# VinAIResearch/Point-Unet

Measured on AMD Instinct MI355X. Metric: points_per_sec_forward, higher is better.
Workload: dtype f32

## Files before the change

point-unet_amd/csrc/debug_hooks.h:

```cpp
#ifndef POINTSEG_DEBUG_H
#define POINTSEG_DEBUG_H
#include "../../include/pointseg.h"
#ifdef __cplusplus
extern "C" {
#endif
int ps_debug_knn_host(const float* support, const float* queries, int64_t B, int64_t n_support,
                      int64_t n_queries, int64_t K, int32_t* out_idx);
int ps_debug_kdtree_host(const float* support, int64_t n, int32_t* vind, int32_t* nodes, float* pts,
                         int32_t* root_depth, float* bbox);
int ps_debug_kdtree_device(ps_context* ctx, const float* support, int64_t n, int32_t* vind, int32_t* nodes,
                           float* pts, int32_t* root_depth, float* bbox);
int ps_debug_pack_weights(const float* W, int cin, int cout, int ntb, float* out);
int ps_debug_pack_b3(const float* W, int cin, int cout, uint16_t* out);
int ps_debug_gemm32(ps_context* ctx, int split_bf16, const float* x1, int ld1, int c1, const int32_t* g1, const float* x2, int ld2, int c2,
                    const int32_t* g2, int gm, int gn, const float* W, const float* bias, int64_t R, int cout, int leaky, float* y, int ldy);
int ps_debug_gemm32_plan(ps_context* ctx, int split_bf16, int64_t R, int cin, int cout, int* out4);

int ps_debug_set_tuning(ps_context* ctx, const char* field, double value);
int ps_debug_get_tuning(ps_context* ctx, const char* field, double* value);
int ps_debug_tuning_fields(char* buf, int cap);
int ps_debug_volume_sample_args_size(void);

#ifdef __cplusplus
}
#endif
#endif
```

point-unet_amd/csrc/debug_hooks.hip:

```cpp
#include "common.h"

#include <cstring>
#include <vector>
#include "kdtree_build.h"
#include "kdtree_host.h"
#include "rowgemm.h"
#include "attpool.h"

using namespace ps;

extern "C" int ps_debug_volume_sample_args_size(void) { return (int)sizeof(ps_volume_sample_args); }

extern "C" int ps_debug_pack_weights(const float* W, int cin, int cout, int ntb, float* out)
{
    PS_CHECK(W && out && (ntb == 1 || ntb == 2 || ntb == 4), "ps_debug_pack_weights: bad argument");
    pack_weights(W, cin, cout, ntb, out);
    return PS_OK;
}

extern "C" int ps_debug_pack_b3(const float* W, int cin, int cout, uint16_t* out)
{
    PS_CHECK(W && out && cin > 0 && cin % 32 == 0 && cout > 0 && cout % 32 == 0, "ps_debug_pack_b3: bad argument");
    pack_b3(W, cin, cout, out);
    return PS_OK;
}

extern "C" int ps_debug_gemm32(ps_context* c, int split_bf16, const float* x1, int ld1, int c1, const int32_t* g1, const float* x2, int ld2, int c2,
                               const int32_t* g2, int gm, int gn, const float* W, const float* bias, int64_t R, int cout, int leaky, float* y, int ldy)
{
    PS_CHECK(c && x1 && W && bias && y && R >= 0 && c1 > 0 && c2 >= 0 && cout > 0, "ps_debug_gemm32: bad argument");
    PS_HIP(hipSetDevice(c->device));
    const int cin = c1 + c2;
    PS_CHECK(cin % (split_bf16 ? 16 : 8) == 0 && cout % 32 == 0, "ps_debug_gemm32: cin %% %d and cout %% 32 must be 0", split_bf16 ? 16 : 8);
    std::vector<float> img((size_t)cin * cout * (split_bf16 ? 3 : 2) / 2);
    if (split_bf16) pack_p32b(W, cin, cout, reinterpret_cast<uint16_t*>(img.data()));
    else pack_p32(W, cin, cout, img.data());
    float *d_img = nullptr, *d_bias = nullptr;
    PS_HIP(hipMalloc(reinterpret_cast<void**>(&d_img), img.size() * sizeof(float)));
    PS_HIP(hipMalloc(reinterpret_cast<void**>(&d_bias), sizeof(float) * (size_t)cout));
    PS_HIP(hipMemcpyAsync(d_img, img.data(), img.size() * sizeof(float), hipMemcpyHostToDevice, c->stream));
    PS_HIP(hipMemcpyAsync(d_bias, bias, sizeof(float) * (size_t)cout, hipMemcpyHostToDevice, c->stream));
    PackedLinear L;
    L.cin = cin; L.cout = cout; L.leaky = leaky; L.bias = d_bias;
    if (split_bf16) L.w32b = d_img; else L.w32 = d_img;
    RowSrc s1, s2;
    s1.x = x1; s1.ld = ld1; s1.c = c1; s1.gather = g1; s1.gm = g1 ? gm : 0; s1.gn = g1 ? gn : 0;
    s2.x = x2; s2.ld = ld2; s2.c = c2; s2.gather = g2; s2.gm = g2 ? gm : 0; s2.gn = g2 ? gn : 0;
    int rc = PS_EINVAL;
    if (split_bf16 ? gemm32b_fits(L, s1, s2, R, ldy) : gemm32_fits(L, s1, s2, R, ldy))
        rc = split_bf16 ? gemm32b(c, L, s1, s2, R, y, ldy) : gemm32(c, L, s1, s2, R, y, ldy);
    else
        set_error("ps_debug_gemm32: the shape does not fit the kernel");
    (void)hipStreamSynchronize(c->stream);
    (void)hipFree(d_img);
    (void)hipFree(d_bias);
    return rc;
}

extern "C" int ps_debug_gemm32_plan(ps_context* c, int split_bf16, int64_t R, int cin, int cout, int* out4)
{
    PS_CHECK(c && out4 && R >= 1 && cin > 0 && cout > 0 && cin % (split_bf16 ? 16 : 8) == 0 && cout % 32 == 0, "ps_debug_gemm32_plan: bad argument");
    const Gemm32Plan p = split_bf16 ? gemm32b_plan(c->tune, R, cin, cout) : gemm32_plan(c->tune, R, cin, cout);
    out4[0] = p.rw;
    out4[1] = p.cw;
    out4[2] = p.sk;
    out4[3] = p.pd;
    return PS_OK;
}

static bool is_bool(double v) { return v == 0 || v == 1; }
static bool is_int_in(double v, double lo, double hi) { return v >= lo && v <= hi && v == (double)(int64_t)v; }

#define PS_TUNING_FIELDS(X)                                                \
    X(gemm32b_min_flops, v >= 0 && v <= 1e300)                             \
    X(gemm32b_rw, v == 0 || v == 1 || v == 2)                              \
    X(gemm32b_cw, v == 0 || v == 1 || v == 2)                              \
    X(gemm32_no_sk8, is_bool(v))                                           \
    X(att64_gemm, is_bool(v))                                              \
    X(att64_occ, v == 0 || v == 1 || v == 2)                               \
    X(att_no_split, is_bool(v))                                            \
    X(wgrad_b3_min_rows, is_int_in(v, 0, (double)(1ll << 40)))             \
    X(gemm_b3_min_rows, is_int_in(v, 0, (double)(1ll << 40)))              \
    X(wgrad_wgs, is_int_in(v, 64, 4096))                                   \
    X(bn_slice, is_bool(v))                                                \
    X(inv_bucket, is_bool(v))                                              \
    X(inv_tile, v == 4096 || v == 6144 || v == 8192)                       \
    X(gather_reduce_ordered, is_bool(v))                                   \
    X(maxpool_bwd_ordered, is_bool(v))                                     \
    X(train_act_bf16, is_bool(v))                                          \
    X(train_att_gemm_split, v == -1 || v == 0 || v == 1)                   \
    X(train_att_gemm, is_bool(v))                                          \
    X(train_att128_fwd_gemm, is_bool(v))                                   \
    X(train_fuse_residual, is_bool(v))                                     \
    X(train_merge_syncbn, is_bool(v))                                      \
    X(convbn_max_c, is_int_in(v, 0, 4096))                                 \
    X(convbn_rect_max, is_int_in(v, 0, (double)(1 << 30)))                 \
    X(wgrad_debug, is_bool(v))

extern "C" int ps_debug_set_tuning(ps_context* c, const char* field, double v)
{
    PS_CHECK(c && field, "ps_debug_set_tuning: NULL argument");
#define PS_SET(f, ok)                                                                                 \
    if (std::strcmp(field, #f) == 0) {                                                                \
        PS_CHECK(ok, "ps_debug_set_tuning: %g is not a value %s is compiled for", v, #f);             \
        c->tune.f = static_cast<decltype(c->tune.f)>(v);                                              \
        return PS_OK;                                                                                 \
    }
    PS_TUNING_FIELDS(PS_SET)
#undef PS_SET
    PS_CHECK(false, "ps_debug_set_tuning: no knob named '%s'", field);
}

extern "C" int ps_debug_get_tuning(ps_context* c, const char* field, double* out)
{
    PS_CHECK(c && field && out, "ps_debug_get_tuning: NULL argument");
#define PS_GET(f, ok)                               \
    if (std::strcmp(field, #f) == 0) {              \
        *out = static_cast<double>(c->tune.f);      \
        return PS_OK;                               \
    }
    PS_TUNING_FIELDS(PS_GET)
#undef PS_GET
    PS_CHECK(false, "ps_debug_get_tuning: no knob named '%s'", field);
}

extern "C" int ps_debug_tuning_fields(char* buf, int cap)
{
    static const char names[] =
#define PS_NAME(f, ok) #f "\n"
        PS_TUNING_FIELDS(PS_NAME)
#undef PS_NAME
        ;
    PS_CHECK(buf && cap >= (int)sizeof(names), "ps_debug_tuning_fields: need %d bytes", (int)sizeof(names));
    std::memcpy(buf, names, sizeof(names));
    return PS_OK;
}

extern "C" int ps_debug_kdtree_device(ps_context* c, const float* support, int64_t n, int32_t* vind, int32_t* nodes, float* pts,
                                      int32_t* root_depth, float* bbox)
{
    PS_CHECK(c && support && vind && nodes && pts && root_depth && bbox && n >= 1, "ps_debug_kdtree_device: bad argument");
    PS_HIP(hipSetDevice(c->device));
    PS_TRY(c->stage_in.reserve(sizeof(float) * 3 * (size_t)n));
    PS_HIP(hipMemcpyAsync(c->stage_in.p, support, sizeof(float) * 3 * (size_t)n, hipMemcpyHostToDevice, c->stream));
    TreeSetPlan plan;
    plan.add((int32_t)n);
    for (int pass = 0; pass < 2; ++pass) {
        c->knn_arena.begin(pass == 0);
        plan.carve(c->knn_arena);
        if (pass == 0) PS_TRY(c->knn_arena.buf.reserve(c->knn_arena.off));
    }
    plan.src[0] = c->stage_in.as<float>();
    PS_TRY(build_trees(c, plan));
    int32_t flag[3] = {0, 0, 0};
    PS_HIP(hipMemcpyAsync(flag, plan.d_flags, 12, hipMemcpyDeviceToHost, c->stream));
    PS_HIP(hipStreamSynchronize(c->stream));
    PS_CHECK(flag[1] == 0, "ps_debug_kdtree_device: builder queue overflow");
    TreeMeta m;
    PS_HIP(hipMemcpyAsync(nodes, plan.d_nodes[0], sizeof(int4) * 2 * (size_t)n, hipMemcpyDeviceToHost, c->stream));
    PS_HIP(hipMemcpyAsync(pts, plan.d_pts[0], sizeof(float4) * (size_t)n, hipMemcpyDeviceToHost, c->stream));
    PS_HIP(hipMemcpyAsync(&m, plan.d_meta, sizeof(TreeMeta), hipMemcpyDeviceToHost, c->stream));
    PS_HIP(hipStreamSynchronize(c->stream));
    for (int64_t i = 0; i < n; ++i) std::memcpy(&vind[i], &pts[4 * i + 3], 4);
    root_depth[0] = m.root;
    root_depth[1] = m.depth;
    for (int a = 0; a < 3; ++a) {
        bbox[a] = m.lo[a];
        bbox[3 + a] = m.hi[a];
    }
    return PS_OK;
}
```

point-unet_amd/csrc/regchain.hip:

```cpp
#include <algorithm>

#include "mfma_tile.h"
#include "rowgemm.h"

namespace ps {

struct RcLayer {
    const float* wp;
    const float* bias;
    float* y;
    const float* ex;
    int ca, cb;
    int ta, tb;
    int cout, ot;
    int ks, ntb;
    int ldy, ldex, leaky;
    int w_off, b_off;
};
struct RcArgs {
    const float* x1; const int32_t* g1; int ld1, g1m, g1n;
    const float* x2; const int32_t* g2; int ld2, g2m, g2n;
    int n, R;
    RcLayer l[kChainMaxSteps];
    const float* image;
    int image_floats;
};

template <int N_, int A0_, int B0_, int O0_, int B1_ = 0, int O1_ = 0, int B2_ = 0, int O2_ = 0, int B3_ = 0, int O3_ = 0>
struct RcShape {
    static constexpr int N = N_, A0 = A0_;
    static constexpr int B[4] = {B0_, B1_, B2_, B3_};
    static constexpr int O[4] = {O0_, O1_, O2_, O3_};
    static constexpr int A(int l) { return l == 0 ? A0_ : O[l - 1]; }
    static constexpr int IN(int l) { return A(l) + B[l]; }
    static constexpr int maxt()
    {
        int m = 1;
        for (int l = 0; l < N_; ++l) {
            m = IN(l) > m ? IN(l) : m;
            m = O[l] > m ? O[l] : m;
        }
        return m;
    }
};

template <int T0, int NT, int MT>
__device__ __forceinline__ void rc_load(float (&dst)[MT][4], const float* __restrict__ rowp, int c, bool vec, int g)
{
#pragma unroll
    for (int t = 0; t < NT; ++t) {
        const int ch = t * 16 + 4 * g;
        if (vec) {
            float4 v = make_float4(0.f, 0.f, 0.f, 0.f);
            if (t + 1 < NT || ch < c) v = *reinterpret_cast<const float4*>(rowp + ch);
            dst[T0 + t][0] = v.x; dst[T0 + t][1] = v.y; dst[T0 + t][2] = v.z; dst[T0 + t][3] = v.w;
        } else {
#pragma unroll
            for (int q = 0; q < 4; ++q) dst[T0 + t][q] = (t + 1 < NT || ch + q < c) ? rowp[ch + q] : 0.f;
        }
    }
}

template <class S, int L>
__device__ __forceinline__ void rc_layer(const RcArgs& a, float (&act)[S::maxt()][4], const float* lds, int lane, int g, int row, int rr, bool ok)
{
    if constexpr (L < S::N) {
        constexpr int IT = S::IN(L), OT = S::O[L], TA = S::A(L), TB = S::B[L];
        const RcLayer& y = a.l[L];
        if constexpr (L > 0 && TB > 0) {
            const bool ve = (y.cb & 3) == 0 && (y.ldex & 3) == 0 && (reinterpret_cast<uintptr_t>(y.ex) & 15) == 0;
            rc_load<TA, TB>(act, y.ex + (size_t)rr * y.ldex, y.cb, ve, g);
        }
        f32x4 acc[OT];
#pragma unroll
        for (int to = 0; to < OT; ++to) acc[to] = f32x4{0.f, 0.f, 0.f, 0.f};
        if constexpr (L > 0) __builtin_amdgcn_sched_barrier(0);
        const float* w = lds + y.w_off + lane;
#pragma unroll
        for (int t0 = 0; t0 < OT; t0 += 4) {
#pragma unroll
            for (int ti = 0; ti < IT; ++ti)
#pragma unroll
                for (int q = 0; q < 4; ++q)
#pragma unroll
                    for (int to = t0; to < (t0 + 4 < OT ? t0 + 4 : OT); ++to)
                        acc[to] = __builtin_amdgcn_mfma_f32_16x16x4f32(w[((to * IT + ti) * 4 + q) * 64], act[ti][q], acc[to], 0, 0, 0);
            if (t0 + 4 < OT) __builtin_amdgcn_sched_barrier(0);
        }
        const bool vy = y.y && (y.cout & 3) == 0 && (y.ldy & 3) == 0 && (reinterpret_cast<uintptr_t>(y.y) & 15) == 0;
#pragma unroll
        for (int to = 0; to < OT; ++to) {
            const int ch = to * 16 + 4 * g;
            const float4 b = *reinterpret_cast<const float4*>(lds + y.b_off + ch);
            float v[4] = {acc[to][0] + b.x, acc[to][1] + b.y, acc[to][2] + b.z, acc[to][3] + b.w};
#pragma unroll
            for (int q = 0; q < 4; ++q) {
                if (y.leaky) v[q] = leaky02(v[q]);
                act[to][q] = v[q];
            }
            if (y.y && ok) {
                float* o = y.y + (size_t)row * y.ldy + ch;
                if (vy) {
                    if (to + 1 < OT || ch < y.cout) *reinterpret_cast<float4*>(o) = make_float4(v[0], v[1], v[2], v[3]);
                } else {
#pragma unroll
                    for (int q = 0; q < 4; ++q)
                        if (to + 1 < OT || ch + q < y.cout) o[q] = v[q];
                }
            }
        }
        rc_layer<S, L + 1>(a, act, lds, lane, g, row, rr, ok);
    }
}

__device__ __forceinline__ void rc_stage(const RcArgs& a, float* dst)
{
    for (int l = 0; l < a.n; ++l) {
        const RcLayer& y = a.l[l];
        const int it_n = y.ta + y.tb;
        const int ln = threadIdx.x & 63, q = threadIdx.x >> 6;
        const int i = ln & 15, gg = ln >> 4;
        const int npairs = it_n * y.ot;
        for (int base = 0; base < npairs; base += 8) {
            float v[8];
#pragma unroll
            for (int u = 0; u < 8; ++u) {
                const int pr = base + u;
                v[u] = 0.f;
                if (pr < npairs) {
                    const int ti = pr / y.ot, to = pr - ti * y.ot;
                    int k;
                    bool kok;
                    if (ti < y.ta) { k = ti * 16 + 4 * gg + q; kok = k < y.ca; }
                    else { k = (ti - y.ta) * 16 + 4 * gg + q; kok = k < y.cb; k += y.ca; }
                    const int cblk = to / y.ntb, j = to - cblk * y.ntb;
                    if (kok && to * 16 + i < y.cout) v[u] = y.wp[(((size_t)cblk * y.ks + (k >> 2)) * 64 + ((k & 3) * 16 + i)) * y.ntb + j];
                }
            }
#pragma unroll
            for (int u = 0; u < 8; ++u) {
                const int pr = base + u;
                if (pr < npairs) {
                    const int ti = pr / y.ot, to = pr - ti * y.ot;
                    dst[y.w_off + ((to * it_n + ti) * 4 + q) * 64 + ln] = v[u];
                }
            }
        }
        for (int e = threadIdx.x; e < y.ot * 16; e += 256) dst[y.b_off + e] = e < y.cout ? y.bias[e] : 0.f;
    }
}

__global__ __launch_bounds__(256) void rc_pack_kernel(RcArgs a, float* out) { rc_stage(a, out); }

template <class S>
__global__ __launch_bounds__(256) void regchain_kernel(RcArgs a)
{
    extern __shared__ __attribute__((aligned(16))) float rc_lds[];
    constexpr int MT = S::maxt();
    const int wave = threadIdx.x >> 6, lane = threadIdx.x & 63;
    const int p = lane & 15, g = lane >> 4;
    if (a.image) {
        for (int i = threadIdx.x; i < a.image_floats / 4; i += 256) reinterpret_cast<float4*>(rc_lds)[i] = reinterpret_cast<const float4*>(a.image)[i];
    } else {
        rc_stage(a, rc_lds);
    }
    __syncthreads();

    const bool v1 = (a.l[0].ca & 3) == 0 && (a.ld1 & 3) == 0 && (reinterpret_cast<uintptr_t>(a.x1) & 15) == 0;
    const bool v2 = (a.l[0].cb & 3) == 0 && (a.ld2 & 3) == 0 && (reinterpret_cast<uintptr_t>(a.x2) & 15) == 0;
    const int stride = gridDim.x * 4;
    auto load_inputs = [&](int tile, float (&dst)[MT][4]) {
        const int rr = min(tile * 16 + p, a.R - 1);
        const int s1 = a.g1 ? (a.g1m ? (rr / a.g1m) * a.g1n : 0) + a.g1[rr] : rr;
        rc_load<0, S::A0>(dst, a.x1 + (size_t)s1 * a.ld1, a.l[0].ca, v1, g);
        if constexpr (S::B[0] > 0) {
            const int s2 = a.g2 ? (a.g2m ? (rr / a.g2m) * a.g2n : 0) + a.g2[rr] : rr;
            rc_load<S::A0, S::B[0]>(dst, a.x2 + (size_t)s2 * a.ld2, a.l[0].cb, v2, g);
        }
    };
    int tile = blockIdx.x * 4 + wave;
    float act[MT][4], nxt[MT][4];
    if (tile * 16 < a.R) load_inputs(tile, nxt);
    for (; tile * 16 < a.R; tile += stride) {
#pragma unroll
        for (int t = 0; t < S::IN(0); ++t)
#pragma unroll
            for (int q = 0; q < 4; ++q) act[t][q] = nxt[t][q];
        if ((tile + stride) * 16 < a.R) load_inputs(tile + stride, nxt);
        const int row = tile * 16 + p;
        rc_layer<S, 0>(a, act, rc_lds, lane, g, row, min(row, a.R - 1), row < a.R);
    }
}

static inline int rc_tiles(int c) { return (c + 15) / 16; }

using RcFc0 = RcShape<2, 1, 0, 1, 0, 1>;
using RcEnc0 = RcShape<2, 1, 0, 1, 1, 2>;
using RcOne0 = RcShape<1, 1, 0, 1>;
using RcPair1 = RcShape<2, 2, 0, 2, 0, 4>;
using RcPair1b = RcShape<2, 4, 0, 2, 0, 4>;
using RcEnc1 = RcShape<2, 4, 0, 4, 2, 8>;
using RcPair2 = RcShape<2, 8, 0, 4, 0, 8>;
using RcHead = RcShape<4, 2, 2, 2, 0, 4, 0, 2, 0, 1>;

template <class S>
static bool rc_matches(const RcArgs& a)
{
    if (a.n != S::N) return false;
    for (int l = 0; l < S::N; ++l)
        if (a.l[l].ta != S::A(l) || a.l[l].tb != S::B[l] || a.l[l].ot != S::O[l]) return false;
    return true;
}

static bool rc_build(const ChainStep* steps, int n_steps, const RowSrc& s1, const RowSrc& s2, RcArgs& a, size_t& lds_bytes)
{
    if (n_steps < 1 || n_steps > kChainMaxSteps) return false;
    a = RcArgs{};
    a.x1 = s1.x; a.g1 = s1.gather; a.ld1 = s1.ld; a.g1m = s1.gm; a.g1n = s1.gn;
    a.x2 = s2.x; a.g2 = s2.gather; a.ld2 = s2.ld; a.g2m = s2.gm; a.g2n = s2.gn;
    a.n = n_steps;
    int off = 0, prev = 0;
    for (int i = 0; i < n_steps; ++i) {
        const PackedLinear* L = steps[i].L;
        if (!L || !L->wp || !L->bias) return false;
        if (steps[i].extra.x && (i == 0 || steps[i].extra.gather)) return false;
        RcLayer& y = a.l[i];
        y.wp = L->wp; y.bias = L->bias; y.y = steps[i].y; y.ldy = steps[i].ldy;
        y.ex = i > 0 ? steps[i].extra.x : nullptr; y.ldex = steps[i].extra.ld;
        y.ca = i == 0 ? s1.c : prev;
        y.cb = i == 0 ? s2.c : (steps[i].extra.x ? steps[i].extra.c : 0);
        if (y.ca + y.cb != L->cin) return false;
        y.ta = rc_tiles(y.ca); y.tb = rc_tiles(y.cb);
        y.cout = L->cout; y.ot = rc_tiles(L->cout);
        y.ks = L->ks; y.ntb = L->ntb; y.leaky = L->leaky;
        y.w_off = off; off += y.ot * (y.ta + y.tb) * 256;
        y.b_off = off; off += y.ot * 16;
        prev = L->cout;
    }
    lds_bytes = (size_t)off * sizeof(float);
    return rc_matches<RcFc0>(a) || rc_matches<RcEnc0>(a) || rc_matches<RcOne0>(a) || rc_matches<RcPair1>(a) || rc_matches<RcPair1b>(a) ||
           rc_matches<RcEnc1>(a) || rc_matches<RcPair2>(a) || rc_matches<RcHead>(a);
}

bool regchain_fits(const ChainStep* steps, int n_steps, const RowSrc& s1, const RowSrc& s2)
{
    RcArgs a;
    size_t lds = 0;
    return rc_build(steps, n_steps, s1, s2, a, lds);
}

template <class S>
static int rc_launch(ps_context* c, const RcArgs& a, size_t lds_bytes, int blocks)
{
    size_t& have = c->regchain_lds_attr[reinterpret_cast<const void*>(regchain_kernel<S>)];
    if (lds_bytes > 48 * 1024 && lds_bytes > have) {
        PS_HIP(hipFuncSetAttribute(reinterpret_cast<const void*>(regchain_kernel<S>), hipFuncAttributeMaxDynamicSharedMemorySize, (int)lds_bytes));
        have = lds_bytes;
    }
    hipLaunchKernelGGL(regchain_kernel<S>, dim3(blocks), dim3(256), lds_bytes, c->stream, a);
    return PS_OK;
}

int regchain(ps_context* c, const ChainStep* steps, int n_steps, const RowSrc& s1, const RowSrc& s2, int64_t R, ChainCache* cache)
{
    if (R <= 0) return PS_OK;
    RcArgs a;
    size_t lds_bytes = 0;
    PS_CHECK(rc_build(steps, n_steps, s1, s2, a, lds_bytes), "regchain: not one of the compiled chain shapes");
    PS_CHECK(R < (int64_t)1 << 31, "regchain: too many rows");
    a.R = (int)R;
    if (cache) {
        ChainCache::Entry* hit = nullptr;
        for (auto& e : cache->entries)
            if (e.wp0 == a.l[0].wp && e.wp_last == a.l[n_steps - 1].wp && e.n == n_steps && e.ca == a.l[0].ca && e.cb == a.l[0].cb) hit = &e;
        if (!hit) {
            cache->entries.emplace_back();
            hit = &cache->entries.back();
            hit->wp0 = a.l[0].wp; hit->wp_last = a.l[n_steps - 1].wp; hit->n = n_steps; hit->ca = a.l[0].ca; hit->cb = a.l[0].cb;
            PS_TRY(hit->img.reserve(lds_bytes));
            hipLaunchKernelGGL(rc_pack_kernel, dim3(1), dim3(256), 0, c->stream, a, hit->img.as<float>());
            PS_HIP(hipGetLastError());
        }
        a.image = hit->img.as<float>();
        a.image_floats = (int)(lds_bytes / sizeof(float));
    }
    const int tiles = (int)((R + 15) / 16);
    const int per_cu = std::max(1, std::min(4, (int)(160 * 1024 / std::max<size_t>(lds_bytes, 1))));
    const int blocks = std::max(1, std::min((tiles + 3) / 4, 256 * per_cu));
    if (rc_matches<RcFc0>(a)) PS_TRY(rc_launch<RcFc0>(c, a, lds_bytes, blocks));
    else if (rc_matches<RcEnc0>(a)) PS_TRY(rc_launch<RcEnc0>(c, a, lds_bytes, blocks));
    else if (rc_matches<RcOne0>(a)) PS_TRY(rc_launch<RcOne0>(c, a, lds_bytes, blocks));
    else if (rc_matches<RcPair1>(a)) PS_TRY(rc_launch<RcPair1>(c, a, lds_bytes, blocks));
    else if (rc_matches<RcPair1b>(a)) PS_TRY(rc_launch<RcPair1b>(c, a, lds_bytes, blocks));
    else if (rc_matches<RcEnc1>(a)) PS_TRY(rc_launch<RcEnc1>(c, a, lds_bytes, blocks));
    else if (rc_matches<RcPair2>(a)) PS_TRY(rc_launch<RcPair2>(c, a, lds_bytes, blocks));
    else PS_TRY(rc_launch<RcHead>(c, a, lds_bytes, blocks));
    PS_HIP(hipGetLastError());
    return PS_OK;
}

}
```

point-unet_amd/csrc/rowgemm.h:

```cpp
#pragma once

#include <vector>

#include "common.h"

namespace ps {

struct PackedLinear {
    const float* wp = nullptr;
    const float* wq = nullptr;
    const void* wb = nullptr;
    const float* w32 = nullptr;
    const void* w32b = nullptr;
    const float* bias = nullptr;
    int cin = 0, cout = 0;
    int ks = 0;
    int ntb = 0;
    int cblocks = 0;
    int leaky = 0;
    int accum = 0;
    size_t packed_floats() const { return (size_t)cblocks * ks * 64 * ntb; }
    int nchunks() const { return (cin + 63) / 64; }
    size_t kperm_floats() const { return (size_t)cblocks * nchunks() * 16 * 64 * ntb; }
    size_t bf16_bytes() const { return (size_t)cblocks * nchunks() * 2 * 64 * ntb * 16; }
    int cout_pad() const { return cblocks * ntb * 16; }
};

inline int choose_ntb(int cout) { return cout >= 64 ? 4 : (cout >= 32 ? 2 : 1); }

void pack_weights(const float* W, int cin, int cout, int ntb, float* out);
void pack_weights_kperm(const float* W, int cin, int cout, int ntb, float* out);

struct RowSrc {
    const float* x = nullptr;
    const int32_t* gather = nullptr;
    int ld = 0;
    int c = 0;
    int gm = 0, gn = 0;
};

struct Gemm32Plan {
    int rw = 1, cw = 1, sk = 1, pd = 2;
    int rgroups = 0, cgroups = 0;
};
Gemm32Plan gemm32_plan(const Tuning& tn, int64_t R, int cin, int cout);
Gemm32Plan gemm32b_plan(const Tuning& tn, int64_t R, int cin, int cout);
bool gemm32_fits(const PackedLinear& L, const RowSrc& s1, const RowSrc& s2, int64_t R, int ldy);
int gemm32(ps_context* c, const PackedLinear& L, const RowSrc& s1, const RowSrc& s2, int64_t R, float* y, int ldy);
void pack_p32b(const float* W, int cin, int cout, uint16_t* out);
bool gemm32b_fits(const PackedLinear& L, const RowSrc& s1, const RowSrc& s2, int64_t R, int ldy);
int gemm32b(ps_context* c, const PackedLinear& L, const RowSrc& s1, const RowSrc& s2, int64_t R, float* y, int ldy);

int rowgemm(ps_context* c, const PackedLinear& L, const RowSrc& s1, const RowSrc& s2, int64_t R, float* y, int ldy);

constexpr int kChainMaxC = 96;
constexpr int kChainMaxSteps = 4;
struct ChainStep {
    const PackedLinear* L = nullptr;
    float* y = nullptr;
    int ldy = 0;
    RowSrc extra;
};
bool rowchain_fits(const ChainStep* steps, int n_steps, const RowSrc& s1, const RowSrc& s2);
bool regchain_fits(const ChainStep* steps, int n_steps, const RowSrc& s1, const RowSrc& s2);
struct ChainCache {
    struct Entry { const float* wp0 = nullptr; const float* wp_last = nullptr; int n = 0, ca = 0, cb = 0; DevBuf img; };
    std::vector<Entry> entries;
    void clear()
    {
        for (auto& e : entries) e.img.release();
        entries.clear();
    }
};
int regchain(ps_context* c, const ChainStep* steps, int n_steps, const RowSrc& s1, const RowSrc& s2, int64_t R, ChainCache* cache);
int rowchain(ps_context* c, const ChainStep* steps, int n_steps, const RowSrc& s1, const RowSrc& s2, int64_t R, ChainCache* cache = nullptr);

bool gemm_b3_fits(const Tuning& tn, int64_t R, int64_t K, int64_t N, const float* x, int64_t ldx, bool one_plane);
size_t gemm_b3_plane_bytes(int64_t K, int64_t N);
int gemm_b3(ps_context* c, const float* x, int64_t ldx, const float* w, int64_t sk, int64_t sn, const float* bias, int64_t R, int64_t K, int64_t N, int leaky,
            int accumulate, float* y, int64_t ldy, void* planes, int pack = 1);

}
```

point-unet_amd/csrc/rowgemm.hip:

```cpp
#include "rowgemm.h"

#include <algorithm>
#include <cstdlib>

#include "mfma_tile.h"

namespace ps {

constexpr int kKC = 64;
constexpr int kPitch = 66;

struct RowGemmArgs {
    const float* x1; const int32_t* g1; int ld1, c1; int g1m, g1n;
    const float* x2; const int32_t* g2; int ld2, c2; int g2m, g2n;
    const float* wp; const float* bias;
    float* y; int ldy;
    int cin, cout, ks, R, leaky;
    int accum;
};

template <int NTB, int RT, bool SPLITK>
__global__ __launch_bounds__(256) void rowgemm_direct_kernel(RowGemmArgs a)
{
    using bfrag = typename BFrag<NTB>::type;
// ... 295 lines not shown
                    }
                } else {
                    const bfrag* w = reinterpret_cast<const bfrag*>(wl) + (size_t)c * 16 * 64 + lane;
#pragma unroll
                    for (int i = 0; i < 4; ++i)
#pragma unroll
                        for (int q = 0; q < 4; ++q) {
                            const bfrag b = w[(size_t)(i * 4 + q) * 64];
                            const float av = q == 0 ? cur[c][i].x : (q == 1 ? cur[c][i].y : (q == 2 ? cur[c][i].z : cur[c][i].w));
#pragma unroll
                            for (int j = 0; j < NTB; ++j) acc[j] = __builtin_amdgcn_mfma_f32_16x16x4f32(av, bfrag_get<NTB>(b, j), acc[j], 0, 0, 0);
                        }
                }
            }
#pragma unroll
        for (int j = 0; j < NTB; ++j) {
            const int col = (cb * NTB + j) * 16 + (lane & 15);
            if (col >= a.cout) continue;
#pragma unroll
            for (int r = 0; r < 4; ++r) {
                const int row = row0 + g * 4 + r;
                if (row < a.R) {
                    float v = acc[j][r] + bias[j];
                    if (a.leaky) v = leaky02(v);
                    if (a.accum) v += old[j][r];
                    a.y[(size_t)row * a.ldy + col] = v;
                }
            }
        }
#pragma unroll
        for (int c = 0; c < 2; ++c)
#pragma unroll
            for (int i = 0; i < 4; ++i) cur[c][i] = nxt[c][i];
    }
}

template <int NTB>
__global__ __launch_bounds__(256) void rowgemm_kernel(RowGemmArgs a)
{
    __shared__ float lds[4][16 * kPitch];
    const int wave = threadIdx.x >> 6, lane = threadIdx.x & 63;
    float* tile = lds[wave];
    const int row0 = (blockIdx.x * 4 + wave) * 16;
    if (row0 >= a.R) return;
    const int cb = blockIdx.y;

    int src1 = 0, src2 = 0;
    {
        const int r = row0 + (lane & 15);
        if (r < a.R) {
            src1 = a.g1 ? (a.g1m ? (r / a.g1m) * a.g1n : 0) + a.g1[r] : r;
            src2 = a.g2 ? (a.g2m ? (r / a.g2m) * a.g2n : 0) + a.g2[r] : r;
        }
    }

    f32x4 acc[NTB];
#pragma unroll
    for (int j = 0; j < NTB; ++j) acc[j] = f32x4{0.f, 0.f, 0.f, 0.f};

    using bfrag = typename BFrag<NTB>::type;
    const bfrag* wp = reinterpret_cast<const bfrag*>(a.wp) + (size_t)cb * a.ks * 64 + lane;

    const int arow = lane & 15, ag = lane >> 4;
    for (int k0 = 0; k0 < a.cin; k0 += kKC) {
        const int kc = min(kKC, a.cin - k0);
        const int kc4 = (kc + 3) & ~3;
        for (int e = lane; e < 16 * kc4; e += 64) {
            const int r = e / kc4, k = e - r * kc4;
            const int kg = k0 + k;
            const int sr1 = __shfl(src1, r), sr2 = __shfl(src2, r);
            float v = 0.f;
            if (row0 + r < a.R && k < kc)
                v = kg < a.c1 ? a.x1[(size_t)sr1 * a.ld1 + kg] : a.x2[(size_t)sr2 * a.ld2 + (kg - a.c1)];
            tile[r * kPitch + k] = v;
        }
        wave_lds_sync();
        const int steps = kc4 >> 2;
        const bfrag* wps = wp + (size_t)(k0 >> 2) * 64;
        for (int s = 0; s < steps; ++s) {
            const float av = tile[arow * kPitch + s * 4 + ag];
            const bfrag bv = wps[(size_t)s * 64];
#pragma unroll
            for (int j = 0; j < NTB; ++j) acc[j] = __builtin_amdgcn_mfma_f32_16x16x4f32(av, bfrag_get<NTB>(bv, j), acc[j], 0, 0, 0);
        }
        wave_lds_sync();
    }

#pragma unroll
    for (int j = 0; j < NTB; ++j) {
        const int col = (cb * NTB + j) * 16 + (lane & 15);
        if (col >= a.cout) continue;
        const float b = a.bias ? a.bias[col] : 0.f;
#pragma unroll
        for (int r = 0; r < 4; ++r) {
            const int row = row0 + (lane >> 4) * 4 + r;
            if (row < a.R) {
                float v = acc[j][r] + b;
                if (a.leaky) v = leaky02(v);
                if (a.accum) v += a.y[(size_t)row * a.ldy + col];
                a.y[(size_t)row * a.ldy + col] = v;
            }
        }
    }
}

static bool aligned16(const void* p) { return (reinterpret_cast<uintptr_t>(p) & 15) == 0; }

struct ChainArgs {
    const float* x1; const int32_t* g1; int ld1, c1; int g1m, g1n;
    const float* x2; const int32_t* g2; int ld2, c2; int g2m, g2n;
    int n, R;
    struct Lyr {
        const float* wp; const float* bias; float* y; const float* ex;
        int cout, ks, ntb, cblocks, leaky, ldy, ldex, cex;
        int w_off, w_floats, b_off, b_floats;
    } l[kChainMaxSteps];
    int tile_off;
    int fast_in;
};
constexpr int kChainPitch = kChainMaxC + 2;

template <int NTB>
__device__ __forceinline__ void chain_layer(const float* __restrict__ in, float* __restrict__ out, const float* __restrict__ wl,
                                            const float* __restrict__ bl, const ChainArgs::Lyr& y, int row0, int R, int lane)
{
    using bfrag = typename BFrag<NTB>::type;
    const int arow = lane & 15, ag = lane >> 4;
    for (int cb = 0; cb < y.cblocks; ++cb) {
        f32x4 acc[NTB];
#pragma unroll
        for (int j = 0; j < NTB; ++j) acc[j] = f32x4{0.f, 0.f, 0.f, 0.f};
        const bfrag* wp = reinterpret_cast<const bfrag*>(wl) + (size_t)cb * y.ks * 64 + lane;
        const float* ap = in + arow * kChainPitch + ag;
        int s = 0;
        for (; s + 4 <= y.ks; s += 4) {
            float av[4];
            bfrag bv[4];
#pragma unroll
            for (int u = 0; u < 4; ++u) { av[u] = ap[(s + u) * 4]; bv[u] = wp[(size_t)(s + u) * 64]; }
#pragma unroll
            for (int u = 0; u < 4; ++u)
#pragma unroll
                for (int j = 0; j < NTB; ++j) acc[j] = __builtin_amdgcn_mfma_f32_16x16x4f32(av[u], bfrag_get<NTB>(bv[u], j), acc[j], 0, 0, 0);
        }
        for (; s < y.ks; ++s) {
            const float av = ap[s * 4];
            const bfrag bv = wp[(size_t)s * 64];
#pragma unroll
            for (int j = 0; j < NTB; ++j) acc[j] = __builtin_amdgcn_mfma_f32_16x16x4f32(av, bfrag_get<NTB>(bv, j), acc[j], 0, 0, 0);
        }
#pragma unroll
        for (int j = 0; j < NTB; ++j) {
            const int col = (cb * NTB + j) * 16 + (lane & 15);
            if (col >= y.cout) continue;
            const float b = bl[col];
#pragma unroll
            for (int r = 0; r < 4; ++r) {
                const int rr = ag * 4 + r;
                float v = acc[j][r] + b;
                if (y.leaky) v = leaky02(v);
                out[rr * kChainPitch + col] = v;
                if (y.y && row0 + rr < R) y.y[(size_t)(row0 + rr) * y.ldy + col] = v;
            }
        }
    }
}

__global__ __launch_bounds__(256) void rowchain_kernel(ChainArgs a)
{
    extern __shared__ __attribute__((aligned(16))) float chain_lds[];
    const int wave = threadIdx.x >> 6, lane = threadIdx.x & 63;
    for (int l = 0; l < a.n; ++l) {
        const ChainArgs::Lyr& y = a.l[l];
        for (int i = threadIdx.x; i < y.w_floats; i += 256) chain_lds[y.w_off + i] = y.wp[i];
        for (int i = threadIdx.x; i < y.b_floats; i += 256) chain_lds[y.b_off + i] = y.bias[i];
    }
    __syncthreads();
    float* const tiles = chain_lds + a.tile_off + wave * (2 * 16 * kChainPitch);
    for (int tile = blockIdx.x * 4 + wave; tile * 16 < a.R; tile += gridDim.x * 4) {
        const int row0 = tile * 16;
        float* in = tiles;
        float* out = tiles + 16 * kChainPitch;
        int src1 = 0, src2 = 0;
        {
            const int r = row0 + (lane & 15);
            if (r < a.R) {
                src1 = a.g1 ? (a.g1m ? (r / a.g1m) * a.g1n : 0) + a.g1[r] : r;
                src2 = a.g2 ? (a.g2m ? (r / a.g2m) * a.g2n : 0) + a.g2[r] : r;
            }
        }
        int cur = a.c1 + a.c2;
        if (a.fast_in) {
            const int q_shift = a.fast_in, qn = 1 << q_shift;
            const int c1q = a.c1 >> 2;
            for (int f0 = 0; f0 < 16 * qn; f0 += 4 * 64) {
                float4 v[4];
                int at[4];
#pragma unroll
                for (int u = 0; u < 4; ++u) {
                    const int f = f0 + u * 64 + lane;
                    const bool on = f < 16 * qn;
                    const int r = on ? f >> q_shift : 0, q = f & (qn - 1);
                    const int sr1 = __shfl(src1, r), sr2 = __shfl(src2, r);
                    at[u] = on ? r * kChainPitch + 4 * q : -1;
                    v[u] = make_float4(0.f, 0.f, 0.f, 0.f);
                    if (on && row0 + r < a.R)
                        v[u] = q < c1q ? *reinterpret_cast<const float4*>(a.x1 + (size_t)sr1 * a.ld1 + 4 * q)
                                       : *reinterpret_cast<const float4*>(a.x2 + (size_t)sr2 * a.ld2 + 4 * (q - c1q));
                }
#pragma unroll
                for (int u = 0; u < 4; ++u)
                    if (at[u] >= 0) {
                        float* d = in + at[u];
                        *reinterpret_cast<float2*>(d) = make_float2(v[u].x, v[u].y);
                        *reinterpret_cast<float2*>(d + 2) = make_float2(v[u].z, v[u].w);
                    }
            }
        } else {
            const int kc4 = (cur + 3) & ~3;
            for (int e0 = 0; e0 < 16 * kc4; e0 += 8 * 64) {
                float v[8];
                int at[8];
#pragma unroll
                for (int u = 0; u < 8; ++u) {
                    const int e = e0 + u * 64 + lane;
                    const bool on = e < 16 * kc4;
                    const int r = on ? e / kc4 : 0, k = on ? e - r * kc4 : 0;
                    const int sr1 = __shfl(src1, r), sr2 = __shfl(src2, r);
                    v[u] = 0.f;
                    at[u] = on ? r * kChainPitch + k : -1;
                    if (on && row0 + r < a.R && k < cur) v[u] = k < a.c1 ? a.x1[(size_t)sr1 * a.ld1 + k] : a.x2[(size_t)sr2 * a.ld2 + (k - a.c1)];
                }
#pragma unroll
                for (int u = 0; u < 8; ++u)
                    if (at[u] >= 0) in[at[u]] = v[u];
            }
        }
        for (int l = 0; l < a.n; ++l) {
            const ChainArgs::Lyr& y = a.l[l];
            if (y.ex) {
                const int w4 = ((cur + y.cex + 3) & ~3) - cur;
                for (int e0 = 0; e0 < 16 * w4; e0 += 8 * 64) {
                    float v[8];
                    int at[8];
#pragma unroll
                    for (int u = 0; u < 8; ++u) {
                        const int e = e0 + u * 64 + lane;
                        const bool on = e < 16 * w4;
                        const int r = on ? e / w4 : 0, k = on ? e - r * w4 : 0;
                        at[u] = on ? r * kChainPitch + cur + k : -1;
                        v[u] = (on && row0 + r < a.R && k < y.cex) ? y.ex[(size_t)(row0 + r) * y.ldex + k] : 0.f;
                    }
#pragma unroll
                    for (int u = 0; u < 8; ++u)
                        if (at[u] >= 0) in[at[u]] = v[u];
                }
                cur += y.cex;
            } else if (l > 0 && (cur & 3)) {
                for (int e = lane; e < 16 * (4 - (cur & 3)); e += 64) {
                    const int w = 4 - (cur & 3), r = e / w, k = e - r * w;
                    in[r * kChainPitch + cur + k] = 0.f;
                }
            }
            wave_lds_sync();
            switch (y.ntb) {
                case 1: chain_layer<1>(in, out, chain_lds + y.w_off, chain_lds + y.b_off, y, row0, a.R, lane); break;
                case 2: chain_layer<2>(in, out, chain_lds + y.w_off, chain_lds + y.b_off, y, row0, a.R, lane); break;
                default: chain_layer<4>(in, out, chain_lds + y.w_off, chain_lds + y.b_off, y, row0, a.R, lane); break;
            }
            wave_lds_sync();
            float* t = in; in = out; out = t;
            cur = y.cout;
        }
    }
}


static bool lds_chain_fits(const ChainStep* steps, int n_steps, const RowSrc& s1, const RowSrc& s2);

bool rowchain_fits(const ChainStep* steps, int n_steps, const RowSrc& s1, const RowSrc& s2)
{
    return regchain_fits(steps, n_steps, s1, s2) || lds_chain_fits(steps, n_steps, s1, s2);
}

static bool lds_chain_fits(const ChainStep* steps, int n_steps, const RowSrc& s1, const RowSrc& s2)
{
    if (n_steps < 1 || n_steps > kChainMaxSteps) return false;
    int cur = s1.c + s2.c;
    for (int i = 0; i < n_steps; ++i) {
        const PackedLinear* L = steps[i].L;
        if (!L || !L->wp) return false;
        cur += steps[i].extra.x ? steps[i].extra.c : 0;
        if (cur != L->cin || ((cur + 3) & ~3) > kChainMaxC || L->cout > kChainMaxC) return false;
        if (steps[i].extra.x && steps[i].extra.gather) return false;
        cur = L->cout;
    }
    return true;
}

int rowchain(ps_context* c, const ChainStep* steps, int n_steps, const RowSrc& s1, const RowSrc& s2, int64_t R, ChainCache* cache)
{
    if (R <= 0) return PS_OK;
    if (regchain_fits(steps, n_steps, s1, s2)) return regchain(c, steps, n_steps, s1, s2, R, cache);
    PS_CHECK(lds_chain_fits(steps, n_steps, s1, s2), "rowchain: the layer chain does not fit (channels above %d or mismatched)", kChainMaxC);
    PS_CHECK(R < (int64_t)1 << 31, "rowchain: too many rows");
    ChainArgs a = {};
    a.x1 = s1.x; a.g1 = s1.gather; a.ld1 = s1.ld; a.c1 = s1.c; a.g1m = s1.gm; a.g1n = s1.gn;
    a.x2 = s2.x; a.g2 = s2.gather; a.ld2 = s2.ld; a.c2 = s2.c; a.g2m = s2.gm; a.g2n = s2.gn;
    a.n = n_steps;
    a.R = (int)R;
    int off = 0;
    for (int i = 0; i < n_steps; ++i) {
        const PackedLinear& L = *steps[i].L;
        ChainArgs::Lyr& y = a.l[i];
        y.wp = L.wp; y.bias = L.bias; y.y = steps[i].y; y.ldy = steps[i].ldy;
        y.ex = steps[i].extra.x; y.ldex = steps[i].extra.ld; y.cex = steps[i].extra.x ? steps[i].extra.c : 0;
        y.cout = L.cout; y.ks = L.ks; y.ntb = L.ntb; y.cblocks = L.cblocks; y.leaky = L.leaky;
        y.w_off = off; y.w_floats = (int)L.packed_floats(); off += (y.w_floats + 3) & ~3;
        y.b_off = off; y.b_floats = L.cout_pad(); off += (y.b_floats + 3) & ~3;
    }
    a.tile_off = off;
    {
        const int cin0 = s1.c + s2.c, q = cin0 / 4;
        const bool pow2 = cin0 % 4 == 0 && q >= 2 && (q & (q - 1)) == 0;
        const bool al = s1.c % 4 == 0 && s2.c % 4 == 0 && s1.ld % 4 == 0 && (s2.c == 0 || s2.ld % 4 == 0) && aligned16(s1.x) && (s2.c == 0 || aligned16(s2.x));
        a.fast_in = 0;
        if (pow2 && al)
            while ((1 << a.fast_in) < q) ++a.fast_in;
    }
    const size_t lds_bytes = sizeof(float) * ((size_t)off + 4 * 2 * 16 * kChainPitch);
    PS_CHECK(lds_bytes <= 160 * 1024, "rowchain: weights of the chain do not fit the LDS (%zu bytes)", lds_bytes);
    if (lds_bytes > c->chain_lds_attr) {
        PS_HIP(hipFuncSetAttribute(reinterpret_cast<const void*>(rowchain_kernel), hipFuncAttributeMaxDynamicSharedMemorySize, (int)lds_bytes));
        c->chain_lds_attr = lds_bytes;
    }
    const int tiles = (int)((R + 15) / 16);
    const int per_cu = std::max(1, (int)(160 * 1024 / lds_bytes));
    const int blocks = std::max(1, std::min((tiles + 3) / 4, 256 * std::min(per_cu, 4)));
    hipLaunchKernelGGL(rowchain_kernel, dim3(blocks), dim3(256), lds_bytes, c->stream, a);
    PS_HIP(hipGetLastError());
    return PS_OK;
}

void pack_weights(const float* W, int cin, int cout, int ntb, float* out)
{
    const int ks = (cin + 3) / 4;
    const int cblocks = (cout + 16 * ntb - 1) / (16 * ntb);
    for (int cb = 0; cb < cblocks; ++cb)
        for (int s = 0; s < ks; ++s)
            for (int l = 0; l < 64; ++l)
                for (int j = 0; j < ntb; ++j) {
                    const int k = s * 4 + (l >> 4);
                    const int col = (cb * ntb + j) * 16 + (l & 15);
                    const float v = (k < cin && col < cout) ? W[(size_t)k * cout + col] : 0.f;
                    out[(((size_t)cb * ks + s) * 64 + l) * ntb + j] = v;
                }
}

void pack_weights_kperm(const float* W, int cin, int cout, int ntb, float* out)
{
    const int nc = (cin + 63) / 64;
    const int cblocks = (cout + 16 * ntb - 1) / (16 * ntb);
    for (int cb = 0; cb < cblocks; ++cb)
        for (int c = 0; c < nc; ++c)
            for (int s = 0; s < 16; ++s)
                for (int l = 0; l < 64; ++l)
                    for (int j = 0; j < ntb; ++j) {
                        const int k = c * 64 + 16 * (l >> 4) + s;
                        const int col = (cb * ntb + j) * 16 + (l & 15);
                        const float v = (k < cin && col < cout) ? W[(size_t)k * cout + col] : 0.f;
                        out[((((size_t)cb * nc + c) * 16 + s) * 64 + l) * ntb + j] = v;
                    }
}


int rowgemm(ps_context* c, const PackedLinear& L, const RowSrc& s1, const RowSrc& s2, int64_t R, float* y, int ldy)
{
    if (R <= 0) return PS_OK;
    PS_CHECK(s1.c + s2.c == L.cin, "rowgemm: sources give %d channels, layer expects %d", s1.c + s2.c, L.cin);
    if (c->att_bf16x3 && 2.0 * (double)R * L.cin * L.cout >= c->tune.gemm32b_min_flops && gemm32b_fits(L, s1, s2, R, ldy))
        return gemm32b(c, L, s1, s2, R, y, ldy);
    if (gemm32_fits(L, s1, s2, R, ldy)) return gemm32(c, L, s1, s2, R, y, ldy);
    PS_CHECK(R < (1ll << 31), "rowgemm: too many rows");
    RowGemmArgs a;
    a.x1 = s1.x; a.g1 = s1.gather; a.ld1 = s1.ld; a.c1 = s1.c; a.g1m = s1.gm; a.g1n = s1.gn;
    a.x2 = s2.x; a.g2 = s2.gather; a.ld2 = s2.ld; a.c2 = s2.c; a.g2m = s2.gm; a.g2n = s2.gn;
    a.wp = L.wp; a.bias = L.bias;
    a.y = y; a.ldy = ldy;
    a.cin = L.cin; a.cout = L.cout; a.ks = L.ks; a.R = (int)R; a.leaky = L.leaky;
    a.accum = L.accum;

    const bool direct = (L.wq || L.wb) && L.cin % 16 == 0 && s1.c % 16 == 0 && s1.ld % 4 == 0 && aligned16(s1.x) &&
                        (s2.c == 0 || (s2.ld % 4 == 0 && aligned16(s2.x)));
    const bool stream = direct && !s1.gather && s2.c == 0 && L.cin <= 128 && ((R + 15) / 16) * L.cblocks >= 32768;
    if (stream) {
        a.wp = L.wb ? static_cast<const float*>(L.wb) : L.wq;
        const dim3 grid(1024, L.cblocks);
#define PS_STREAM(NTB)                                                                                                      \
    if (L.wb) hipLaunchKernelGGL((rowgemm_stream_kernel<NTB, true>), grid, dim3(256), 0, c->stream, a);                       \
    else hipLaunchKernelGGL((rowgemm_stream_kernel<NTB, false>), grid, dim3(256), 0, c->stream, a)
        switch (L.ntb) {
            case 1: PS_STREAM(1); break;
            case 2: PS_STREAM(2); break;
            case 4: PS_STREAM(4); break;
            default: set_error("rowgemm: bad ntb %d", L.ntb); return PS_EINVAL;
        }
#undef PS_STREAM
    } else if (direct && L.wb) {
        a.wp = static_cast<const float*>(L.wb);
        const int64_t tiles16 = (R + 15) / 16;
        const bool rt2 = tiles16 * L.cblocks >= 8192;
#define PS_LAUNCH_BF(NTB, RT, GX) hipLaunchKernelGGL((rowgemm_direct_bf16_kernel<NTB, RT>), dim3((unsigned)(GX), L.cblocks), dim3(256), 0, c->stream, a)
#define PS_BF_BY_NTB(RT, GX)                                                 \
    switch (L.ntb) {                                                         \
        case 1: PS_LAUNCH_BF(1, RT, GX); break;                              \
        case 2: PS_LAUNCH_BF(2, RT, GX); break;                              \
        case 4: PS_LAUNCH_BF(4, RT, GX); break;                              \
        default: set_error("rowgemm: bad ntb %d", L.ntb); return PS_EINVAL;  \
    }
        if (rt2) {
            PS_BF_BY_NTB(2, (tiles16 + 7) / 8)
        } else {
            PS_BF_BY_NTB(1, (tiles16 + 3) / 4)
        }
#undef PS_BF_BY_NTB
#undef PS_LAUNCH_BF
    } else if (direct) {
        a.wp = L.wq;
        const int64_t tiles16 = (R + 15) / 16;
        const bool splitk = L.cin >= 256 && tiles16 * L.cblocks < 2048;
        const bool rt2 = !splitk && tiles16 * L.cblocks >= 8192;
#define PS_LAUNCH(NTB, RT, SK, GX)                                                                                             \
    hipLaunchKernelGGL((rowgemm_direct_kernel<NTB, RT, SK>), dim3((unsigned)(GX), L.cblocks), dim3(256), 0, c->stream, a)
#define PS_BY_NTB(RT, SK, GX)                                    \
    switch (L.ntb) {                                             \
        case 1: PS_LAUNCH(1, RT, SK, GX); break;                 \
        case 2: PS_LAUNCH(2, RT, SK, GX); break;                 \
        case 4: PS_LAUNCH(4, RT, SK, GX); break;                 \
        default: set_error("rowgemm: bad ntb %d", L.ntb); return PS_EINVAL; \
    }
        if (splitk) {
            PS_BY_NTB(1, true, tiles16)
        } else if (rt2) {
            PS_BY_NTB(2, false, (tiles16 + 7) / 8)
        } else {
            PS_BY_NTB(1, false, (tiles16 + 3) / 4)
        }
#undef PS_BY_NTB
#undef PS_LAUNCH
    } else {
        dim3 grid(ceil_div(R, 64), L.cblocks);
        switch (L.ntb) {
            case 1: hipLaunchKernelGGL(rowgemm_kernel<1>, grid, dim3(256), 0, c->stream, a); break;
            case 2: hipLaunchKernelGGL(rowgemm_kernel<2>, grid, dim3(256), 0, c->stream, a); break;
            case 4: hipLaunchKernelGGL(rowgemm_kernel<4>, grid, dim3(256), 0, c->stream, a); break;
            default: set_error("rowgemm: bad ntb %d", L.ntb); return PS_EINVAL;
        }
    }
    PS_HIP(hipGetLastError());
    return PS_OK;
}

}
```

Before: 190.5 million.

## Use 8-wave blocks for RcEnc1 regchain and overlap weight staging with input loads

Templates the register-chain kernel on wave count and launches the RcEnc1 chain shape with 8 waves (512 threads) per block instead of 4, so each block's large LDS weight image is shared by more row tiles. For the cached-image path with more than four waves, the weight-image copy into LDS is unrolled eight float4 loads deep and the first tile's input loads are issued before the LDS stores. This is meant to hide global-memory latency behind the staging copy. It also adds a debug entry point and a grid_limit parameter for testing chain paths. The change may cost occupancy or register pressure, and grid sizing now divides tiles by eight for that shape.

```diff
diff --git a/point-unet_amd/csrc/debug_hooks.h b/point-unet_amd/csrc/debug_hooks.h
--- a/point-unet_amd/csrc/debug_hooks.h
+++ b/point-unet_amd/csrc/debug_hooks.h
@@ -16,6 +16,10 @@
                     const int32_t* g2, int gm, int gn, const float* W, const float* bias, int64_t R, int cout, int leaky, float* y, int ldy);
 int ps_debug_gemm32_plan(ps_context* ctx, int split_bf16, int64_t R, int cin, int cout, int* out4);
 
+int ps_debug_chain(ps_context* ctx, int path, int n_steps, const float* x1, int ld1, int c1, const int32_t* g1, const float* x2, int ld2, int c2,
+                   const int32_t* g2, int gm, int gn, const float* const* W, const float* const* bias, const int* cout, const int* leaky,
+                   float* const* y, const int* ldy, int ex_step, const float* ex, int ldex, int cex, int64_t R, int cached, int grid_limit);
+
 int ps_debug_set_tuning(ps_context* ctx, const char* field, double value);
 int ps_debug_get_tuning(ps_context* ctx, const char* field, double* value);
 int ps_debug_tuning_fields(char* buf, int cap);
diff --git a/point-unet_amd/csrc/debug_hooks.hip b/point-unet_amd/csrc/debug_hooks.hip
--- a/point-unet_amd/csrc/debug_hooks.hip
+++ b/point-unet_amd/csrc/debug_hooks.hip
@@ -57,6 +57,62 @@
     return rc;
 }
 
+extern "C" int ps_debug_chain(ps_context* c, int path, int n_steps, const float* x1, int ld1, int c1, const int32_t* g1, const float* x2, int ld2, int c2,
+                              const int32_t* g2, int gm, int gn, const float* const* W, const float* const* bias, const int* cout, const int* leaky,
+                              float* const* y, const int* ldy, int ex_step, const float* ex, int ldex, int cex, int64_t R, int cached, int grid_limit)
+{
+    PS_CHECK(c && x1 && W && bias && cout && leaky && y && ldy && n_steps >= 1 && n_steps <= kChainMaxSteps && R >= 0 && c1 > 0 && c2 >= 0 && grid_limit >= 0,
+             "ps_debug_chain: bad argument");
+    PS_HIP(hipSetDevice(c->device));
+    PackedLinear L[kChainMaxSteps];
+    ChainStep st[kChainMaxSteps];
+    std::vector<float> host;
+    size_t w_off[kChainMaxSteps], b_off[kChainMaxSteps];
+    int cin = c1 + c2;
+    for (int i = 0; i < n_steps; ++i) {
+        if (ex && i == ex_step) cin += cex;
+        PS_CHECK(W[i] && bias[i] && cout[i] > 0, "ps_debug_chain: bad layer %d", i);
+        L[i].cin = cin; L[i].cout = cout[i]; L[i].leaky = leaky[i];
+        L[i].ks = (cin + 3) / 4;
+        L[i].ntb = choose_ntb(cout[i]);
+        L[i].cblocks = (cout[i] + 16 * L[i].ntb - 1) / (16 * L[i].ntb);
+        w_off[i] = (host.size() + 63) & ~size_t(63);
+        host.resize(w_off[i] + L[i].packed_floats());
+        pack_weights(W[i], cin, cout[i], L[i].ntb, host.data() + w_off[i]);
+        b_off[i] = (host.size() + 63) & ~size_t(63);
+        host.resize(b_off[i] + (size_t)L[i].cout_pad());
+        for (int k = 0; k < L[i].cout_pad(); ++k) host[b_off[i] + k] = k < cout[i] ? bias[i][k] : 0.f;
+        cin = cout[i];
+    }
+    float* d = nullptr;
+    PS_HIP(hipMalloc(reinterpret_cast<void**>(&d), host.size() * sizeof(float)));
+    int rc = hipMemcpyAsync(d, host.data(), host.size() * sizeof(float), hipMemcpyHostToDevice, c->stream) == hipSuccess ? PS_OK : PS_EHIP;
+    for (int i = 0; i < n_steps; ++i) {
+        L[i].wp = d + w_off[i]; L[i].bias = d + b_off[i];
+        st[i].L = &L[i]; st[i].y = y[i]; st[i].ldy = ldy[i];
+        if (ex && i == ex_step) { st[i].extra.x = ex; st[i].extra.ld = ldex; st[i].extra.c = cex; }
+    }
+    RowSrc s1, s2;
+    s1.x = x1; s1.ld = ld1; s1.c = c1; s1.gather = g1; s1.gm = g1 ? gm : 0; s1.gn = g1 ? gn : 0;
+    s2.x = x2; s2.ld = ld2; s2.c = c2; s2.gather = g2; s2.gm = g2 ? gm : 0; s2.gn = g2 ? gn : 0;
+    if (rc == PS_OK) {
+        ChainCache cache;
+        if (path == 0 && !regchain_fits(st, n_steps, s1, s2)) {
+            set_error("ps_debug_chain: not one of the compiled chain shapes");
+            rc = PS_EINVAL;
+        } else {
+            rc = path == 0 ? regchain(c, st, n_steps, s1, s2, R, cached ? &cache : nullptr, grid_limit)
+                           : rowchain_lds(c, st, n_steps, s1, s2, R);
+        }
+        (void)hipStreamSynchronize(c->stream);
+        cache.clear();
+    } else {
+        set_error("ps_debug_chain: upload failed");
+    }
+    (void)hipFree(d);
+    return rc;
+}
+
 extern "C" int ps_debug_gemm32_plan(ps_context* c, int split_bf16, int64_t R, int cin, int cout, int* out4)
 {
     PS_CHECK(c && out4 && R >= 1 && cin > 0 && cout > 0 && cin % (split_bf16 ? 16 : 8) == 0 && cout % 32 == 0, "ps_debug_gemm32_plan: bad argument");
diff --git a/point-unet_amd/csrc/regchain.hip b/point-unet_amd/csrc/regchain.hip
--- a/point-unet_amd/csrc/regchain.hip
+++ b/point-unet_amd/csrc/regchain.hip
@@ -152,23 +152,17 @@
 
 __global__ __launch_bounds__(256) void rc_pack_kernel(RcArgs a, float* out) { rc_stage(a, out); }
 
-template <class S>
-__global__ __launch_bounds__(256) void regchain_kernel(RcArgs a)
+template <class S, int WAVES>
+__global__ __launch_bounds__(WAVES * 64) void regchain_kernel(RcArgs a)
 {
     extern __shared__ __attribute__((aligned(16))) float rc_lds[];
-    constexpr int MT = S::maxt();
+    constexpr int MT = S::maxt(), NT = WAVES * 64;
     const int wave = threadIdx.x >> 6, lane = threadIdx.x & 63;
     const int p = lane & 15, g = lane >> 4;
-    if (a.image) {
-        for (int i = threadIdx.x; i < a.image_floats / 4; i += 256) reinterpret_cast<float4*>(rc_lds)[i] = reinterpret_cast<const float4*>(a.image)[i];
-    } else {
-        rc_stage(a, rc_lds);
-    }
-    __syncthreads();
 
     const bool v1 = (a.l[0].ca & 3) == 0 && (a.ld1 & 3) == 0 && (reinterpret_cast<uintptr_t>(a.x1) & 15) == 0;
     const bool v2 = (a.l[0].cb & 3) == 0 && (a.ld2 & 3) == 0 && (reinterpret_cast<uintptr_t>(a.x2) & 15) == 0;
-    const int stride = gridDim.x * 4;
+    const int stride = gridDim.x * WAVES;
     auto load_inputs = [&](int tile, float (&dst)[MT][4]) {
         const int rr = min(tile * 16 + p, a.R - 1);
         const int s1 = a.g1 ? (a.g1m ? (rr / a.g1m) * a.g1n : 0) + a.g1[rr] : rr;
@@ -178,9 +172,41 @@
             rc_load<S::A0, S::B[0]>(dst, a.x2 + (size_t)s2 * a.ld2, a.l[0].cb, v2, g);
         }
     };
-    int tile = blockIdx.x * 4 + wave;
+    int tile = blockIdx.x * WAVES + wave;
     float act[MT][4], nxt[MT][4];
-    if (tile * 16 < a.R) load_inputs(tile, nxt);
+    if (a.image && WAVES > 4) {
+        const float4* src = reinterpret_cast<const float4*>(a.image);
+        float4* dst = reinterpret_cast<float4*>(rc_lds);
+        const int n4 = a.image_floats / 4;
+#define RC_ROUND(X) X(0) X(1) X(2) X(3) X(4) X(5) X(6) X(7)
+#define RC_LD(u) const float4 v##u = src[min(base + u * NT, n4 - 1)];
+#define RC_ST(u) dst[min(base + u * NT, n4 - 1)] = v##u;
+        {
+            const int base = threadIdx.x;
+            RC_ROUND(RC_LD)
+            if (tile * 16 < a.R) load_inputs(tile, nxt);
+            __builtin_amdgcn_sched_barrier(0);
+            RC_ROUND(RC_ST)
+        }
+        for (int base = threadIdx.x + NT * 8; base < n4; base += NT * 8) {
+            RC_ROUND(RC_LD)
+            __builtin_amdgcn_sched_barrier(0);
+            RC_ROUND(RC_ST)
+        }
+#undef RC_ST
+#undef RC_LD
+#undef RC_ROUND
+        __syncthreads();
+    } else {
+        if (a.image) {
+            for (int i = threadIdx.x; i < a.image_floats / 4; i += NT) reinterpret_cast<float4*>(rc_lds)[i] = reinterpret_cast<const float4*>(a.image)[i];
+        } else if (threadIdx.x < 256) {
+            rc_stage(a, rc_lds);
+        }
+        __syncthreads();
+        if (tile * 16 < a.R) load_inputs(tile, nxt);
+    }
+
     for (; tile * 16 < a.R; tile += stride) {
 #pragma unroll
         for (int t = 0; t < S::IN(0); ++t)
@@ -249,19 +275,24 @@
     return rc_build(steps, n_steps, s1, s2, a, lds);
 }
 
-template <class S>
-static int rc_launch(ps_context* c, const RcArgs& a, size_t lds_bytes, int blocks)
-{
-    size_t& have = c->regchain_lds_attr[reinterpret_cast<const void*>(regchain_kernel<S>)];
+template <class S, int WAVES>
+static int rc_launch(ps_context* c, const RcArgs& a, size_t lds_bytes, int grid_limit)
+{
+    const void* fn = reinterpret_cast<const void*>(regchain_kernel<S, WAVES>);
+    size_t& have = c->regchain_lds_attr[fn];
     if (lds_bytes > 48 * 1024 && lds_bytes > have) {
-        PS_HIP(hipFuncSetAttribute(reinterpret_cast<const void*>(regchain_kernel<S>), hipFuncAttributeMaxDynamicSharedMemorySize, (int)lds_bytes));
+        PS_HIP(hipFuncSetAttribute(fn, hipFuncAttributeMaxDynamicSharedMemorySize, (int)lds_bytes));
         have = lds_bytes;
     }
-    hipLaunchKernelGGL(regchain_kernel<S>, dim3(blocks), dim3(256), lds_bytes, c->stream, a);
+    const int tiles = (a.R + 15) / 16;
+    const int per_cu = std::max(1, std::min(4, (int)(160 * 1024 / std::max<size_t>(lds_bytes, 1))));
+    int blocks = std::max(1, std::min((tiles + WAVES - 1) / WAVES, 256 * per_cu));
+    if (grid_limit > 0) blocks = std::min(blocks, grid_limit);
+    hipLaunchKernelGGL((regchain_kernel<S, WAVES>), dim3(blocks), dim3(WAVES * 64), lds_bytes, c->stream, a);
     return PS_OK;
 }
 
-int regchain(ps_context* c, const ChainStep* steps, int n_steps, const RowSrc& s1, const RowSrc& s2, int64_t R, ChainCache* cache)
+int regchain(ps_context* c, const ChainStep* steps, int n_steps, const RowSrc& s1, const RowSrc& s2, int64_t R, ChainCache* cache, int grid_limit)
 {
     if (R <= 0) return PS_OK;
     RcArgs a;
@@ -284,17 +315,14 @@
         a.image = hit->img.as<float>();
         a.image_floats = (int)(lds_bytes / sizeof(float));
     }
-    const int tiles = (int)((R + 15) / 16);
-    const int per_cu = std::max(1, std::min(4, (int)(160 * 1024 / std::max<size_t>(lds_bytes, 1))));
-    const int blocks = std::max(1, std::min((tiles + 3) / 4, 256 * per_cu));
-    if (rc_matches<RcFc0>(a)) PS_TRY(rc_launch<RcFc0>(c, a, lds_bytes, blocks));
-    else if (rc_matches<RcEnc0>(a)) PS_TRY(rc_launch<RcEnc0>(c, a, lds_bytes, blocks));
-    else if (rc_matches<RcOne0>(a)) PS_TRY(rc_launch<RcOne0>(c, a, lds_bytes, blocks));
-    else if (rc_matches<RcPair1>(a)) PS_TRY(rc_launch<RcPair1>(c, a, lds_bytes, blocks));
-    else if (rc_matches<RcPair1b>(a)) PS_TRY(rc_launch<RcPair1b>(c, a, lds_bytes, blocks));
-    else if (rc_matches<RcEnc1>(a)) PS_TRY(rc_launch<RcEnc1>(c, a, lds_bytes, blocks));
-    else if (rc_matches<RcPair2>(a)) PS_TRY(rc_launch<RcPair2>(c, a, lds_bytes, blocks));
-    else PS_TRY(rc_launch<RcHead>(c, a, lds_bytes, blocks));
+    if (rc_matches<RcFc0>(a)) PS_TRY((rc_launch<RcFc0, 4>(c, a, lds_bytes, grid_limit)));
+    else if (rc_matches<RcEnc0>(a)) PS_TRY((rc_launch<RcEnc0, 4>(c, a, lds_bytes, grid_limit)));
+    else if (rc_matches<RcOne0>(a)) PS_TRY((rc_launch<RcOne0, 4>(c, a, lds_bytes, grid_limit)));
+    else if (rc_matches<RcPair1>(a)) PS_TRY((rc_launch<RcPair1, 4>(c, a, lds_bytes, grid_limit)));
+    else if (rc_matches<RcPair1b>(a)) PS_TRY((rc_launch<RcPair1b, 4>(c, a, lds_bytes, grid_limit)));
+    else if (rc_matches<RcEnc1>(a)) PS_TRY((rc_launch<RcEnc1, 8>(c, a, lds_bytes, grid_limit)));
+    else if (rc_matches<RcPair2>(a)) PS_TRY((rc_launch<RcPair2, 4>(c, a, lds_bytes, grid_limit)));
+    else PS_TRY((rc_launch<RcHead, 4>(c, a, lds_bytes, grid_limit)));
     PS_HIP(hipGetLastError());
     return PS_OK;
 }
diff --git a/point-unet_amd/csrc/rowgemm.h b/point-unet_amd/csrc/rowgemm.h
--- a/point-unet_amd/csrc/rowgemm.h
+++ b/point-unet_amd/csrc/rowgemm.h
@@ -72,8 +72,9 @@
         entries.clear();
     }
 };
-int regchain(ps_context* c, const ChainStep* steps, int n_steps, const RowSrc& s1, const RowSrc& s2, int64_t R, ChainCache* cache);
+int regchain(ps_context* c, const ChainStep* steps, int n_steps, const RowSrc& s1, const RowSrc& s2, int64_t R, ChainCache* cache, int grid_limit = 0);
 int rowchain(ps_context* c, const ChainStep* steps, int n_steps, const RowSrc& s1, const RowSrc& s2, int64_t R, ChainCache* cache = nullptr);
+int rowchain_lds(ps_context* c, const ChainStep* steps, int n_steps, const RowSrc& s1, const RowSrc& s2, int64_t R);
 
 bool gemm_b3_fits(const Tuning& tn, int64_t R, int64_t K, int64_t N, const float* x, int64_t ldx, bool one_plane);
 size_t gemm_b3_plane_bytes(int64_t K, int64_t N);
diff --git a/point-unet_amd/csrc/rowgemm.hip b/point-unet_amd/csrc/rowgemm.hip
--- a/point-unet_amd/csrc/rowgemm.hip
+++ b/point-unet_amd/csrc/rowgemm.hip
@@ -621,6 +621,12 @@
 {
     if (R <= 0) return PS_OK;
     if (regchain_fits(steps, n_steps, s1, s2)) return regchain(c, steps, n_steps, s1, s2, R, cache);
+    return rowchain_lds(c, steps, n_steps, s1, s2, R);
+}
+
+int rowchain_lds(ps_context* c, const ChainStep* steps, int n_steps, const RowSrc& s1, const RowSrc& s2, int64_t R)
+{
+    if (R <= 0) return PS_OK;
     PS_CHECK(lds_chain_fits(steps, n_steps, s1, s2), "rowchain: the layer chain does not fit (channels above %d or mismatched)", kChainMaxC);
     PS_CHECK(R < (int64_t)1 << 31, "rowchain: too many rows");
     ChainArgs a = {};
```

After: 191.0 million (median of 6 runs). No clear change (+0.3%).
